# jwmak/ceres-solver-cuda

Hardware: AMD Instinct MI355X
Metric: residual+Jacobian evaluations/sec on BAL problem-13682; achieved HBM GB/s (higher is better)
Workload: dtype f64

## Files before the change

__graft_entry__.py:

```python
import os
import subprocess
import sys

REPO = os.path.dirname(os.path.abspath(__file__))
PKG = os.path.join(REPO, "ceres-solver-cuda_amd")
for p in (PKG, os.path.join(REPO, "oracle"), os.path.join(REPO, "tests")):
    if p not in sys.path:
        sys.path.insert(0, p)


def build():
    jobs = str(min(16, os.cpu_count() or 1))
    subprocess.check_call(["make", "-j", jobs, "-C", PKG])
    subprocess.check_call(["make", "-j", jobs, "-C", os.path.join(REPO, "examples")])
    subprocess.check_call(["make", "-j", jobs, "-C", os.path.join(REPO, "oracle")])
    subprocess.check_call(["make", "-j", jobs, "-C", os.path.join(REPO, "tests", "hip")])
    subprocess.check_call(["make", "-j", jobs, "-C", os.path.join(REPO, "tests", "cpp"),
                           "all", "asan-cpu", "asan-hip"])
    subprocess.check_call(["make", "-j", jobs, "-C", os.path.join(REPO, "tests", "cpp"),
                           "-f", "per_block_loss.mk", "driver", "facade"])
    subprocess.check_call(["make", "-j", jobs, "-C", os.path.join(REPO, "tests", "cpp"),
                           "-f", "schur_pairs.mk", "driver"])
    subprocess.check_call(["make", "-j", jobs, "-C", os.path.join(REPO, "tests", "cpp"),
                           "-f", "schur_sparse.mk", "driver"])
    subprocess.check_call(["make", "-j", jobs, "-C", os.path.join(REPO, "tests", "cpp"),
                           "-f", "cg_state.mk", "driver"])
    import ceres_amd
    from ceres_amd import _cse
    _cse.lib()
    return ceres_amd


def smoke():
    import numpy as np
    import torch

    import ceres_amd as ca
    from ceres_amd import bal
    import oracle_py as O
    from parity_util import assert_parity

    assert torch.cuda.is_available(), "smoke() needs a HIP device"
    prog = bal.synthetic_program((16, 2000, 7600), loss=ca.Loss.huber(1.0), seed=11)
    ev = ca.Evaluator(prog, device=0)
    got = ev.evaluate()
    info = ev.info()
    ev.close()
    op = O.OracleProgram.from_program(prog)
    ref = op.evaluate(prog.state, num_threads=4)
    assert_parity(got, ref, "smoke")
    assert info.num_affine_groups == 1
    print(f"smoke ok: cost {got[1]:.12e} (oracle {ref[1]:.12e}), "
          f"{prog.num_residual_blocks} blocks, {prog.num_jacobian_values} Jacobian values")
    return True


if __name__ == "__main__":
    build()
    if len(sys.argv) > 1 and sys.argv[1] == "smoke":
# ... 2 lines not shown
```

ceres-solver-cuda_amd/ceres_amd/_cse.py:

```python
import ctypes as C
import os

HERE = os.path.dirname(os.path.abspath(__file__))
LIB_PATH = os.path.normpath(os.path.join(HERE, "..", "lib", "libcse.so"))

CSE_ABI_VERSION = 6

JACOBIAN_CLOSED_FORM = 0
JACOBIAN_JET = 1
CSE_OK = 0
CSE_EVALUATION_FAILED = 1
CSE_ERR_INVALID = -1
CSE_ERR_HIP = -2
CSE_ERR_OOM = -3
CSE_ERR_UNSUPPORTED = -4
EVAL_SAME_POINT = 1

SNAVELY_2_9_3 = 0
SNAVELY_NO_DISTORTION_2_7_3 = 1
SNAVELY_QUATERNION_2_10_3 = 2
POINT_DISPLACEMENT_3_3 = 3
TEST_LINEAR_3_2_3_4 = 100
TEST_LINEAR_3_4_3_2 = 101
TEST_LINEAR_2_2_3 = 102
# ... 138 lines not shown
    "cse_set_plus_jacobians": (C.c_int, [C.c_void_p, P_f64]),
    "cse_plus_device": (C.c_int, [C.c_void_p, C.c_void_p, C.c_void_p, C.c_void_p]),
    "cse_plus": (C.c_int, [C.c_void_p, P_f64, P_f64, P_f64]),
    "cse_jacobian_right_multiply": (C.c_int, [C.c_void_p, C.c_void_p, C.c_void_p, C.c_void_p]),
    "cse_jacobian_left_multiply": (C.c_int, [C.c_void_p, C.c_void_p, C.c_void_p, C.c_void_p]),
    "cse_cgnr_multiply": (C.c_int, [C.c_void_p, C.c_void_p, C.c_void_p, C.c_void_p, C.c_void_p]),
    "cse_jacobian_squared_column_norm": (C.c_int, [C.c_void_p, C.c_void_p, C.c_void_p]),
    "cse_jacobian_scale_columns": (C.c_int, [C.c_void_p, C.c_void_p, C.c_void_p]),
    "cse_schur_structure": (C.c_int, [C.c_void_p, P_i64, P_i64]),
    "cse_schur_init": (C.c_int, [C.c_void_p, C.c_void_p, C.c_void_p, C.c_void_p, C.c_void_p,
                                 C.c_int]),
    "cse_schur_init_gradient": (C.c_int, [C.c_void_p, C.c_void_p, C.c_void_p, C.c_void_p,
                                          C.c_void_p, C.c_int, C.c_void_p]),
    "cse_schur_multiply": (C.c_int, [C.c_void_p, C.c_void_p, C.c_void_p]),
    "cse_schur_precondition": (C.c_int, [C.c_void_p, C.c_void_p, C.c_void_p]),
    "cse_schur_back_substitute": (C.c_int, [C.c_void_p, C.c_void_p, C.c_void_p]),
    "cse_schur_complement": (C.c_int, [C.c_void_p, C.c_void_p, C.c_int64]),
    "cse_schur_complement_plan": (C.c_int, [C.c_void_p, P_i64, P_i64, P_i64]),
    "cse_schur_complement_sparse_structure": (C.c_int, [C.c_void_p, P_i64, P_i64, P_i64, P_i64, P_i32]),
    "cse_schur_complement_sparse": (C.c_int, [C.c_void_p, C.c_void_p]),
    "cse_schur_explicit_multiply": (C.c_int, [C.c_void_p, C.c_void_p, C.c_void_p, C.c_void_p]),
    "cse_cg_default_options": (None, [C.POINTER(cse_cg_options)]),
    "cse_schur_solve": (C.c_int, [C.c_void_p, C.POINTER(cse_cg_options), C.c_void_p, C.c_void_p,
                                  C.c_void_p, C.c_void_p, C.POINTER(cse_cg_summary)]),
    "cse_create_multi": (C.c_int, [C.POINTER(cse_problem_desc), C.POINTER(cse_options),
                                   P_i32, C.c_int32, C.POINTER(C.c_void_p)]),
    "cse_shard_info": (C.c_int, [C.c_void_p, P_i32, P_i64, P_i32]),
    "cse_shard_transfer_bytes": (C.c_int, [C.c_void_p, P_i64, P_i64]),
    "cse_host_register": (C.c_int, [C.c_void_p, C.c_size_t]),
    "cse_host_unregister": (C.c_int, [C.c_void_p]),
    "cse_destroy": (None, [C.c_void_p]),
    "cse_last_error": (C.c_char_p, []),
    "cse_get_info": (C.c_int, [C.c_void_p, C.POINTER(cse_info)]),
    "cse_kernel_stats": (C.c_int, [C.c_void_p, P_f64, P_f64, P_i64]),
    "cse_reset_kernel_stats": (C.c_int, [C.c_void_p]),
    "cse_block_sparse_layout": (C.c_int, [C.c_int64, P_pb, C.c_int64, P_i64, P_i32, P_i32,
                                          C.c_int64, P_i64, P_i64, P_i64, P_i64]),
    "cse_compressed_row_layout": (C.c_int, [C.c_int64, P_pb, C.c_int64, P_i64, P_i32, P_i32,
                                            P_i64, P_i64, P_i64, P_i64, P_i64, P_i64]),
    "cse_layout_offsets_count": (C.c_int64, [C.c_int64, P_pb, C.c_int64, P_i64, P_i32, P_i32]),
    "cse_register_functor": (C.c_int, [C.c_void_p, P_i32]),
    "cse_functor_shape": (C.c_int, [C.c_int32, P_i32, P_i32, P_i32, P_i32]),
    "cse_abi_version": (C.c_int, []),
    "cse_build_info": (C.c_char_p, []),
}

_SINCE_ROUND3 = {"cse_evaluate_ex", "cse_evaluate_device_ex"}
_DEFAULT_LIB = LIB_PATH

_lib = None


def use_library(path):
    global LIB_PATH
    if _lib is not None:
        raise RuntimeError("libcse already loaded from " + LIB_PATH)
    LIB_PATH = os.path.abspath(path)


def lib():
    global _lib
    if _lib is None:
        if not os.path.exists(LIB_PATH):
            raise RuntimeError(
                f"libcse.so not found at {LIB_PATH}: build it with `make -C "
                f"ceres-solver-cuda_amd` (there is no CPU fallback)")
        handle = C.CDLL(LIB_PATH)
        for name, (res, args) in SIGNATURES.items():
            if name in _SINCE_ROUND3 and LIB_PATH != _DEFAULT_LIB and not hasattr(handle, name):
                continue
            fn = getattr(handle, name)
            fn.restype = res
            fn.argtypes = args
        if handle.cse_abi_version() != CSE_ABI_VERSION:
            raise RuntimeError("libcse.so ABI version mismatch")
        _lib = handle
    return _lib


def cg_options(**fields):
    o = cse_cg_options()
    lib().cse_cg_default_options(C.byref(o))
    for k, v in fields.items():
        if k not in dict(cse_cg_options._fields_):
            raise TypeError(f"cse_cg_options has no field {k}")
        setattr(o, k, v)
    return o


def last_error():
    return lib().cse_last_error().decode()


def functor_shape(kind):
    if kind in FUNCTOR_SHAPES:
        return FUNCTOR_SHAPES[kind]
    nr, nb, d = C.c_int32(), C.c_int32(), C.c_int32()
    sizes = (C.c_int32 * MAX_PARAMETER_BLOCKS)()
    check(lib().cse_functor_shape(int(kind), C.byref(nr), C.byref(nb), sizes, C.byref(d)),
          "cse_functor_shape")
    shape = (nr.value, tuple(sizes[:nb.value]), d.value)
    FUNCTOR_SHAPES[kind] = shape
# ... 13 lines not shown
```

ceres-solver-cuda_amd/ceres_amd/problem.py:

```python
import ctypes as C
from dataclasses import dataclass, field
from typing import List, Optional

import numpy as np

from . import _cse
from ._cse import FUNCTOR_SHAPES, functor_shape

BLOCK_SPARSE = "block_sparse"
COMPRESSED_ROW = "compressed_row"


def _ptr(a, ctype):
    if a is None:
        return None
    return a.ctypes.data_as(C.POINTER(ctype))


@dataclass
class Loss:
    kind: int = _cse.LOSS_TRIVIAL
    a: float = 1.0
    scaled: bool = False
    scale: float = 1.0
# ... 436 lines not shown
        forms = {"closed": _cse.JACOBIAN_CLOSED_FORM, "jet": _cse.JACOBIAN_JET}
        if jacobian_form not in forms:
            raise ValueError(f"jacobian_form must be one of {sorted(forms)}")
        opts.jacobian_form = forms[jacobian_form]
        opts.use_stream = int(stream is not None)
        opts.stream = stream if stream else None
        h = C.c_void_p()
        if devices is None:
            _cse.check(L.cse_create(C.byref(self.desc), C.byref(opts), C.byref(h)), "cse_create")
        else:
            if stream is not None:
                raise ValueError("a multi-device evaluator runs on its own per-device streams")
            devs = (C.c_int32 * len(devices))(*devices)
            _cse.check(L.cse_create_multi(C.byref(self.desc), C.byref(opts), devs, len(devices),
                                          C.byref(h)), "cse_create_multi")
        self.handle = h

    def close(self):
        if getattr(self, "handle", None):
            _cse.lib().cse_destroy(self.handle)
            self.handle = None

    def __del__(self):
        try:
            self.close()
        except Exception:
            pass

    def info(self):
        inf = _cse.cse_info()
        _cse.check(_cse.lib().cse_get_info(self.handle, C.byref(inf)), "cse_get_info")
        return inf

    def shard_info(self):
        L = _cse.lib()
        n = C.c_int32()
        _cse.check(L.cse_shard_info(self.handle, C.byref(n), None, None), "cse_shard_info")
        first = np.empty(n.value + 1, np.int64)
        devs = np.empty(n.value, np.int32)
        _cse.check(L.cse_shard_info(self.handle, C.byref(n), _ptr(first, C.c_int64),
                                    _ptr(devs, C.c_int32)), "cse_shard_info")
        return first, devs

    def transfer_bytes(self):
        first, _ = self.shard_info()
        n = len(first) - 1
        h2d = np.empty(n, np.int64)
        d2h = np.empty(n, np.int64)
        _cse.check(_cse.lib().cse_shard_transfer_bytes(self.handle, _ptr(h2d, C.c_int64),
                                                        _ptr(d2h, C.c_int64)),
                   "cse_shard_transfer_bytes")
        return h2d, d2h

    def evaluate(self, state=None, residuals=True, gradient=True, jacobian=True, out=None,
                 new_evaluation_point=True):
        p = self.program
        state = np.ascontiguousarray(p.state if state is None else state, np.float64)
        cost = C.c_double(-1.0)
        ro, go, jo = out if out is not None else (None, None, None)
        r = (ro if ro is not None else np.empty(p.num_residuals)) if residuals else None
        g = (go if go is not None else np.empty(p.num_effective_parameters)) if gradient else None
        j = (jo if jo is not None else np.empty(p.num_jacobian_values)) if jacobian else None
        flags = 0 if new_evaluation_point else _cse.EVAL_SAME_POINT
        rc = _cse.lib().cse_evaluate_ex(self.handle, _ptr(state, C.c_double), C.byref(cost),
                                        _ptr(r, C.c_double), _ptr(g, C.c_double),
                                        _ptr(j, C.c_double), flags)
# ... 140 lines not shown
```

ceres-solver-cuda_amd/csrc/cse_evaluator.hip:

```cpp
#include <hip/hip_runtime.h>

#include <algorithm>
#include <cmath>
#include <cstdio>
#include <cstdlib>
#include <cstring>
#include <mutex>
#include <new>
#include <string>
#include <type_traits>
#include <utility>
#include <vector>

#include "../../include/cse.h"
#include "evaluation_kernels.hpp"
#include "evaluator.hpp"
#include "group_store_kernel.hpp"
#include "jet_kernels.h"
#include "kernel_pickers.hpp"
#include "launch.hpp"
#include "multi_device.h"
#include "per_block_loss_kernels.h"
#include "plan.hpp"

// ... 132 lines not shown
    a.jac_stride[j] = G.jac_stride[j];
    for (int r = 0; r < 3; ++r) a.jac_base[j][r] = G.jac_base[j][r];
  }
  a.res_base = G.res_base;
  a.packed0 = G.packed0.p;
  a.packed0_lo = G.slot0_lo;
  a.packed0_stride = G.packed_stride;
  a.act0_bits = G.act0.p;
  a.fbase = G.fbase.p;
  a.side = G.side.p;
  a.delta0 = G.delta0.p;
  a.gindex = G.gindex.p;
  a.first = G.first;
  a.residual_layout = ev->res_layout.p;
  a.jac_layout = ev->jac_layout.p;
  a.jac_offsets = ev->jac_offsets.p;
  a.residuals = res;
  a.jacobian = jac;
  a.gradient = grad;
  a.partials = ev->partials.p + G.partial_offset;
  a.status = ev->status.p;
  a.loss.a = G.loss.a;
  a.loss.scale = G.loss.scale;
  a.loss.scaled = G.loss.scaled;
  static_assert(sizeof(a.user_loss) == sizeof(G.loss.user), "user loss bytes");
  std::memcpy(a.user_loss, G.loss.user, sizeof(a.user_loss));
  a.apply_loss = ev->opts.apply_loss_function;
  a.check_finite = ev->opts.check_finite;
  a.table_runs = G.runs.p;
  a.plain0 = G.plain0 ? 1 : 0;
  a.plain0_state_base = G.plain0_state_base;
  a.plain0_delta_base = G.plain0_delta_base;
  a.loss_data = G.loss_data.p;
  return a;
}

cse::GradArgs SlotGradArgs(const Group& G, int j, const double* jac, const double* res, double* grad) {
  const Group::GradPlan& P = G.grad[j];
  cse::GradArgs ga{};
  ga.jac = jac;
  for (int r = 0; r < G.shape.nr && r < 3; ++r) ga.jrow[r] = G.jac_base[j][r];
  ga.jstride = G.jac_stride[j];
  ga.res = res;
  ga.res_base = G.res_base;
  ga.perm = P.perm.p;
  ga.off = P.off.p;
  ga.count = P.count;
  ga.lo = P.lo;
  ga.grad = grad;
  ga.delta_base = G.delta_base[j];
  return ga;
}

int LaunchContribReduce(const Group::GradPlan& P, const double* gcontrib, const cse::GradArgs& ga,
                        hipStream_t s) {
  const cse::GradChunks ch = GradChunksOf(P);
  if (P.nchunks > 0)
    hipLaunchKernelGGL((cse::GradientContribKernel<9, 10>),
                       dim3((unsigned)((P.nchunks + cse::kWavesPerBlock - 1) / cse::kWavesPerBlock)),
                       dim3(cse::kBlockThreads), 0, s, gcontrib, P.perm.p, ch, P.chunk_order.p);
  hipLaunchKernelGGL((cse::GradientChunkReduceKernel<9>),
                     dim3((unsigned)((ga.count + cse::kBlockThreads - 1) / cse::kBlockThreads)),
                     dim3(cse::kBlockThreads), 0, s, ga, ch);
  CSE_HIP(hipGetLastError());
  return CSE_OK;
}
// ... 124 lines not shown
    return Fail(CSE_ERR_UNSUPPORTED, "fused gradient: slot 0 of " + std::to_string(G.shape.s0) + " parameters");
  CSE_HIP(hipGetLastError());
  return CSE_OK;
}

int UploadGroup(const cse_residual_group& g, const cse::GroupTables& T, Group* Gp, hipStream_t s) {
  Group& G = *Gp;
  const KindShape& k = G.shape;
  int rc;
  if (G.repack0 && (rc = G.packed0.alloc((size_t)G.slot0_count * G.packed_stride))) return rc;
  if ((rc = G.act0.upload(T.bits.data(), T.bits.size(), s))) return rc;
  if ((rc = G.src0.upload(T.src.data(), T.src.size(), s))) return rc;
  if ((rc = G.delta0.upload(T.dlt.data(), T.dlt.size(), s))) return rc;
  if ((rc = G.fbase.upload(T.fbase.data(), T.fbase.size(), s))) return rc;
  if ((rc = G.prev_seg.upload(T.prev_seg.data(), T.prev_seg.size(), s))) return rc;
  if ((rc = G.side.alloc(T.prev_seg.size() * 16))) return rc;
  for (int j = 0; j < 2; ++j) {
    Group::GradPlan& D = G.grad[j];
    const cse::GradTables& H = T.grad[j];
    static_cast<cse::GradPlanInfo&>(D) = T.grad_info[j];
    if ((rc = D.perm.upload(H.perm.data(), H.perm.size(), s))) return rc;
    if ((rc = D.off.upload(H.off.data(), H.off.size(), s))) return rc;
    if ((rc = D.chunk_order.upload(H.chunk_order.data(), H.chunk_order.size(), s))) return rc;
    if ((rc = D.chunk_begin.upload(H.chunk_begin.data(), H.chunk_begin.size(), s))) return rc;
    if ((rc = D.chunk_off.upload(H.chunk_off.data(), H.chunk_off.size(), s))) return rc;
    if ((rc = D.chunk_pb.upload(H.chunk_pb.data(), H.chunk_pb.size(), s))) return rc;
    const int size = j == 0 ? k.s0 : k.s1;
    if (D.ready && !D.sorted &&
        (rc = D.chunk_partial.alloc((size_t)std::max<int64_t>(1, D.nchunks) * size)))
      return rc;
  }
  if ((rc = G.runs.upload(T.runs.data(), T.runs.size(), s))) return rc;
  if ((rc = G.ids.upload(g.parameter_block_ids, (size_t)g.num_blocks * k.nb, s))) return rc;
  std::vector<double> rows, records;
  if (G.loss_data_size) {
    const int64_t n = g.num_blocks, D = k.data, W = D + G.loss_data_size;
    rows.resize((size_t)(n * D));
    records.resize((size_t)(n * 2));
    for (int64_t i = 0; i < n; ++i) {
      for (int64_t c = 0; c < D; ++c) rows[i * D + c] = g.functor_data[i * W + c];
      records[2 * i] = g.functor_data[i * W + D];
      records[2 * i + 1] = g.functor_data[i * W + D + 1];
    }
    if ((rc = G.data.upload(rows.data(), rows.size(), s))) return rc;
    if ((rc = G.loss_data.upload(records.data(), records.size(), s))) return rc;
  } else if ((rc = G.data.upload(g.functor_data, (size_t)g.num_blocks * k.data, s))) {
    return rc;
  }
  if ((!G.affine || G.const0) && g.residual_block_index &&
      (rc = G.gindex.upload(g.residual_block_index, (size_t)g.num_blocks, s)))
    return rc;
  if (hipStreamSynchronize(s) != hipSuccess) return Fail(CSE_ERR_HIP, "upload failed");
  return CSE_OK;
}

struct GradPath {
  bool grad_pass = false, fused = false, recompute = false;
};
bool FusedGradMode(const cse_evaluator* ev, const Group& G) {
  const int mode = ev->opts.gradient_mode;
  return G.fuse_ok && (mode == 0 || (!G.user && ((mode == 3 && !G.jet) || (mode == 1 && G.const0))));
}
GradPath GradPathOf(const cse_evaluator* ev, const Group& G, bool grad, bool res, bool jac) {
  GradPath p;
  p.grad_pass = grad && res && jac && G.affine && ev->opts.gradient_mode != 2;
  for (int j = 0; j < G.shape.nb; ++j) p.grad_pass = p.grad_pass && G.grad[j].ready;
// ... 539 lines not shown

int cse_functor_shape(int32_t kind, int32_t* num_residuals, int32_t* num_parameter_blocks,
                      int32_t* parameter_block_sizes, int32_t* data_size) {
  KindShape k;
  if (!ShapeOf(kind, &k)) return Fail(CSE_ERR_UNSUPPORTED, "unknown functor kind " + std::to_string(kind));
  if (num_residuals) *num_residuals = k.nr;
  if (num_parameter_blocks) *num_parameter_blocks = k.nb;
  if (parameter_block_sizes)
    for (int j = 0; j < k.nb; ++j) parameter_block_sizes[j] = k.sz[j];
  if (data_size) *data_size = k.data;
  return CSE_OK;
}

int cse_get_info(cse_evaluator* ev, cse_info* info) {
  if (!ev || !info) return Fail(CSE_ERR_INVALID, "null argument");
  if (ev->multi) return MultiInfo(ev->multi, info);
  std::memset(info, 0, sizeof(*info));
  info->num_residual_blocks = ev->num_residual_blocks;
  info->num_residuals = ev->num_residuals;
  info->num_parameters = ev->num_parameters;
  info->num_effective_parameters = ev->num_effective;
  info->num_jacobian_values = ev->num_jacobian_values;
  info->num_groups = (int32_t)ev->groups.size();
  for (auto& G : ev->groups) {
    info->num_affine_groups += G.affine ? 1 : 0;
    info->num_fused_gradient_groups += FusedGradMode(ev, G) ? 1 : 0;
  }
  info->device = ev->device;
  info->bytes_jacobian_eval = ev->bytes_jac;
  info->bytes_residual_eval = ev->bytes_res;
  return CSE_OK;
}

int cse_kernel_stats(cse_evaluator* ev, double* last_ms, double* total_ms, int64_t* launches) {
  if (!ev) return Fail(CSE_ERR_INVALID, "null evaluator");
  if (ev->multi) return MultiKernelStats(ev->multi, last_ms, total_ms, launches);
  if (!ev->opts.profile) return Fail(CSE_ERR_INVALID, "evaluator created without options.profile");
  int rc = FoldTiming(ev);
  if (rc) return rc;
  if (last_ms) *last_ms = ev->last_ms;
  if (total_ms) *total_ms = ev->total_ms;
  if (launches) *launches = ev->launches;
  return CSE_OK;
}

int cse_reset_kernel_stats(cse_evaluator* ev) {
  if (!ev) return Fail(CSE_ERR_INVALID, "null evaluator");
  if (ev->multi) return MultiResetKernelStats(ev->multi);
  int rc = FoldTiming(ev);
  if (rc) return rc;
  ev->last_ms = ev->total_ms = 0.0;
  ev->launches = 0;
  return CSE_OK;
}

}
```

ceres-solver-cuda_amd/csrc/evaluate_kernel.hpp:

```cpp
#ifndef CSE_EVALUATE_KERNEL_HPP_
#define CSE_EVALUATE_KERNEL_HPP_

#include <type_traits>

#include "kernel_common.hpp"

namespace cse {

template <class K, bool kJac, bool kCrs, bool kHalves = false, bool kConst0 = false>
__device__ __forceinline__ void StageAndStore(const GroupArgs& a, double* st, int lane, bool active,
                                              int64_t i0, int nw, const double* r,
                                              const double* J0, const double* J1,
                                              bool act0 = true, int64_t c = 0) {
  using Tr = KindTraits<K>;
  constexpr int NR = Tr::NR, NB = Tr::NB, S0 = Tr::S0, S1 = Tr::S1, S1p = Tr::S1p;
  constexpr int N = S0 + S1;
  if (nw <= 0) return;
  if (a.residuals && active) {
    double* dst = a.residuals + a.res_base + (int64_t)NR * (i0 + lane);
#pragma unroll
    for (int k = 0; k < NR; ++k) __builtin_nontemporal_store(r[k], dst + k);
  }
  if constexpr (kJac) {
    if (!a.jacobian) return;
// ... 96 lines not shown
  }
}

template <int kR, int kCols>
__device__ __forceinline__ void AddGradientSlot(double* g, int t, const double* r, const double* J) {
#pragma unroll
  for (int c = 0; c < kCols; ++c) {
    if (c >= t) break;
    double s = 0.0;
#pragma unroll
    for (int k = 0; k < kR; ++k) s += J[k * kCols + c] * r[k];
    unsafeAtomicAdd(g + c, s);
  }
}

template <class K>
struct AffineInputs {
  double d[KindTraits<K>::D];
  double x0[KindTraits<K>::X0];
  double x0pad;
  double x1[KindTraits<K>::S1p];
  int32_t id0, id1;
};

template <class K>
__device__ __forceinline__ int2 LoadIds(const GroupArgs& a, int64_t i) {
  if constexpr (KindTraits<K>::NB == 2) {
    return *reinterpret_cast<const int2*>(a.ids + 2 * i);
  } else {
    return make_int2(a.ids[i], 0);
  }
}

template <class K, bool kNtLoads>
__device__ __forceinline__ void GatherDataAndSlot1(const GroupArgs& a, int64_t i, int2 id,
                                                   AffineInputs<K>* in) {
  using Tr = KindTraits<K>;
  constexpr int S1 = Tr::S1, D = Tr::D;
  if constexpr (kNtLoads) {
#pragma unroll
    for (int k = 0; k < D; ++k) in->d[k] = __builtin_nontemporal_load(a.data + i * D + k);
  } else if constexpr (D == 2) {
    const double2 v = *reinterpret_cast<const double2*>(a.data + 2 * i);
    in->d[0] = v.x;
    in->d[1] = v.y;
  } else {
#pragma unroll
    for (int k = 0; k < D; ++k) in->d[k] = a.data[i * D + k];
  }
  if constexpr (S1 > 0) {
    const double* p1 = a.state + a.state_base[1] + (int64_t)S1 * id.y;
#pragma unroll
    for (int k = 0; k < S1; ++k) in->x1[k] = kNtLoads ? __builtin_nontemporal_load(p1 + k) : p1[k];
  }
}

template <class K>
__device__ __forceinline__ void GatherCoop(const GroupArgs& a, int64_t i, int2 id,
                                           AffineInputs<K>* in, double* lds, int lane) {
  constexpr int X0 = KindTraits<K>::X0;
  GatherDataAndSlot1<K, false>(a, i, id, in);
  const double* base0 = a.state + a.state_base[0];
  double piece[X0];
#pragma unroll
  for (int k = 0; k < X0; ++k) {
    const int p = k * kWave + lane;
// ... 10 lines not shown
  in->id0 = id.x;
  in->id1 = id.y;
}

template <class K>
__device__ __forceinline__ void GatherCoopDma(const GroupArgs& a, int64_t i, int2 id,
                                              AffineInputs<K>* in, double* lds, int lane) {
  using Tr = KindTraits<K>;
  constexpr int X0 = Tr::X0;
  constexpr int X0p = (X0 + 1) & ~1;
  constexpr int kPieces = X0p / 2;
  constexpr int kRow = PackedRowDoubles(X0);
  const int cid_own = id.x - a.packed0_lo;
#pragma unroll
  for (int k = 0; k < kPieces; ++k) {
    const int p = k * kWave + lane;
    const int t = p / kPieces, q = p - t * kPieces;
    const int cid = __shfl(cid_own, t, kWave);
    const double* src = a.packed0 + (int64_t)kRow * cid + 2 * q;
    __builtin_amdgcn_global_load_lds(src, lds + 2 * kWave * k, 16, 0, 0);
  }
  GatherDataAndSlot1<K, true>(a, i, id, in);
  asm volatile("s_waitcnt vmcnt(0)" ::: "memory");
  __builtin_amdgcn_wave_barrier();
#pragma unroll
  for (int k = 0; k < X0; ++k) in->x0[k] = lds[lane * X0p + k];
  if constexpr (X0 < X0p) in->x0pad = lds[lane * X0p + X0];
  __builtin_amdgcn_wave_barrier();
  in->id0 = id.x;
  in->id1 = id.y;
}

template <class K>
__device__ __forceinline__ void GatherEarly(const GroupArgs& a, int64_t i, int2 id,
                                            AffineInputs<K>* in, double* lds, int lane) {
  using Tr = KindTraits<K>;
  constexpr int X0 = Tr::X0, S1 = Tr::S1, D = Tr::D;
  constexpr int X0p = (X0 + 1) & ~1;
  constexpr int kPieces = X0p / 2;
  static_assert(D == 2, "observation pairs");
  const double obs_x = __builtin_nontemporal_load(a.data + 2 * i);
  const double obs_y = __builtin_nontemporal_load(a.data + 2 * i + 1);
  const int cid_own = id.x - a.packed0_lo;
#pragma unroll
  for (int k = 0; k < kPieces; ++k) {
    const int p = k * kWave + lane;
    const int t = p / kPieces, q = p - t * kPieces;
    const int cid = __shfl(cid_own, t, kWave);
    const double* src = a.packed0 + (int64_t)PackedRowDoubles(X0) * cid + 2 * q;
    __builtin_amdgcn_global_load_lds(src, lds + 2 * kWave * k, 16, 0, 0);
  }
  if constexpr (S1 > 0) {
    const double* p1 = a.state + a.state_base[1] + (int64_t)S1 * id.y;
#pragma unroll
    for (int k = 0; k < S1; ++k) in->x1[k] = __builtin_nontemporal_load(p1 + k);
  }
  in->d[0] = obs_x;
  in->d[1] = obs_y;
  asm volatile("s_waitcnt vmcnt(0)" ::: "memory");
  __builtin_amdgcn_wave_barrier();
#pragma unroll
  for (int k = 0; k < X0; ++k) in->x0[k] = lds[lane * X0p + k];
  __builtin_amdgcn_wave_barrier();
  in->id0 = id.x;
  in->id1 = id.y;
}

template <int S>
__device__ __forceinline__ void SegmentedScan(double* v, int key, int lane) {
#pragma unroll
  for (int off = 1; off < kWave; off <<= 1) {
    const int ku = __shfl_up(key, off, kWave);
    double vu[S];
#pragma unroll
    for (int c = 0; c < S; ++c) vu[c] = __shfl_up(v[c], off, kWave);
// ... 192 lines not shown
                          : kCrs ? kStageMinLaneCrs : kStageMinLane;
  constexpr int kStageLane = kPadLane > kStageLane1 ? kPadLane : kStageLane1;
  __shared__ double stage[kWPB][kWave * kStageLane];

  constexpr bool kC0J = T::kConst0 && kJac;
  const int lane = threadIdx.x & (kWave - 1);
  const int wave = kWPB == 1 ? 0 : threadIdx.x / kWave;
  const int64_t num_chunks = (a.n + kWave - 1) / kWave;
  const int64_t c = (int64_t)blockIdx.x * kWPB + wave;
  double* partial_dst = a.partials + c;
  if (c >= num_chunks) {
    if (lane == 0) *partial_dst = 0.0;
    return;
  }
  double* st = stage[wave];
  const int64_t i0 = c * kWave;
  const int64_t rem = a.n - i0;
  const int nw = rem < kWave ? (int)rem : kWave;
  const bool active = lane < nw;
  const int64_t i = active ? i0 + lane : a.n - 1;
  int64_t fb[5] = {0, 0, 0, 0, 0};
  if constexpr (kC0J) {
    fb[0] = a.fbase[c];
    fb[1] = a.fbase[c + 1];
    fb[2] = a.fbase[0];
    fb[3] = a.fbase[num_chunks];
    fb[4] = a.fbase[c + 2 < num_chunks ? c + 2 : num_chunks];
  }

  AffineInputs<K> in;
  LossParams lp;
  LoadBlockLoss<kLoss, kCoop == 2>(a, i, &lp);
  if constexpr (kCoop == 2) {
    int2 id;
    if constexpr (Tr::NB == 2) {
      const long long b = __builtin_nontemporal_load(reinterpret_cast<const long long*>(a.ids) + i);
      id = make_int2((int)b, (int)(b >> 32));
    } else {
      id = LoadIds<K>(a, i);
    }
    if constexpr (!kJac && Tr::D == 2 && Tr::NB == 2) {
      GatherEarly<K>(a, i, id, &in, st, lane);
    } else {
      GatherCoopDma<K>(a, i, id, &in, st, lane);
    }
  } else {
    GatherCoop<K>(a, i, LoadIds<K>(a, i), &in, st, lane);
  }
  if constexpr (kC0J) {
    if constexpr (kWPB == 1)
      asm volatile("" : "+s"(fb[0]), "+s"(fb[1]), "+s"(fb[2]), "+s"(fb[3]), "+s"(fb[4]));
    else
      asm volatile("" : "+v"(fb[0]), "+v"(fb[1]), "+v"(fb[2]), "+v"(fb[3]), "+v"(fb[4]));
  }
  double r[NR], J0[NR * S0], J1[NR * S1p];
  bool ok = EvaluateFunctor<K, kJac>(in.d, in.x0, in.x1, r, J0, J1);
  if (ok && a.check_finite) {
    bool bad = AnyNonFinite<NR>(r);
    if constexpr (kJac) bad = bad || AnyNonFinite<NR * S0>(J0) || AnyNonFinite<NR * S1>(J1);
    ok = !bad;
  }
  const double cost =
      LossAndCorrect<K, kLoss, kJac>(LossOf<kLoss>(a, lp), a.apply_loss, r, J0, J1, a.residuals != nullptr,
                                     a.user_loss);
  bool act0 = true;
  if constexpr (T::kConst0) {
    static_assert(kCoop == 2, "constant slot-0 blocks: the repacked table");
    if constexpr ((Tr::X0 & 1) != 0) {
      act0 = in.x0pad == 0.0;
    } else {
      const uint32_t k0 = (uint32_t)(in.id0 - a.packed0_lo);
      act0 = ((a.act0_bits[k0 >> 5] >> (k0 & 31)) & 1u) != 0;
    }
  }
  if (kJac && a.gradient != nullptr && active) {
    if (act0)
// ... 933 lines not shown
```

ceres-solver-cuda_amd/csrc/evaluator.hpp:

```cpp
#ifndef CSE_EVALUATOR_HPP_
#define CSE_EVALUATOR_HPP_

#include <hip/hip_runtime.h>

#include <cstdint>
#include <string>
#include <utility>
#include <vector>

#include "../../include/cse.h"
#include "cg_state.hpp"
#include "plan.hpp"

struct CseMulti;

namespace cse {

struct GroupArgs;
struct GradArgs;

inline int Fail(int code, const std::string& msg) { return CseFail(code, msg); }

#define CSE_SINGLE_DEVICE(ev, what)                                                         \
  do {                                                                                     \
// ... 32 lines not shown
    if (count == 0) return CSE_OK;
    if (hipMalloc(&p, count * sizeof(T)) != hipSuccess) {
      p = nullptr;
      return Fail(CSE_ERR_OOM, "hipMalloc of " + std::to_string(count * sizeof(T)) + " bytes failed");
    }
    n = count;
    return CSE_OK;
  }
  int ensure(size_t count) {
    if (p && n >= count) return CSE_OK;
    return alloc(count);
  }
  int upload(const T* h, size_t count, hipStream_t s) {
    int rc = alloc(count);
    if (rc) return rc;
    if (count && hipMemcpyAsync(p, h, count * sizeof(T), hipMemcpyHostToDevice, s) != hipSuccess)
      return Fail(CSE_ERR_HIP, "hipMemcpyAsync H2D failed");
    return CSE_OK;
  }
  void release() {
    if (p) (void)hipFree(p);
    p = nullptr;
    n = 0;
  }
};

struct Group : cse::GroupPlan {
  std::string user_name;
  DevBuf<int32_t> ids;
  DevBuf<double> data;
  DevBuf<double> loss_data;
  DevBuf<int64_t> gindex;
  DevBuf<double> packed0;
  struct GradPlan : cse::GradPlanInfo {
    DevBuf<int32_t> perm;
    DevBuf<int64_t> off;
    DevBuf<int64_t> chunk_begin, chunk_off;
    DevBuf<int32_t> chunk_pb;
    DevBuf<int32_t> chunk_order;
    DevBuf<double> chunk_partial;
  } grad[2];
  DevBuf<uint32_t> act0;
  DevBuf<int64_t> src0, fbase, delta0;
  DevBuf<double> side;
  DevBuf<int32_t> prev_seg;
  DevBuf<double> gside, gcontrib;
  DevBuf<double> sdata;
  DevBuf<int32_t> sid1;
  bool sorted_ready = false;
  DevBuf<int64_t> runs;
};

constexpr int kOperatorWavesPerWg = cse::kWavesPerBlock;

inline bool SnavelyShaped(const Group& G) { return cse::SnavelyShaped(G.shape); }
inline bool UserFused(const Group& G) { return cse::UserFused(G.user, G.shape); }

}

struct cse_evaluator {
  CseMulti* multi = nullptr;
  int device = 0;
  int num_cus = 256;
  hipStream_t stream = nullptr;
  bool own_stream = false;
  cse_options opts{};
// ... 73 lines not shown
```

ceres-solver-cuda_amd/csrc/host_shared.hpp:

```cpp
#ifndef CSE_HOST_SHARED_HPP_
#define CSE_HOST_SHARED_HPP_

#include <stdint.h>

namespace cse {

constexpr int kBlockThreads = 256;
constexpr int kWave = 64;
constexpr int kWavesPerBlock = kBlockThreads / kWave;
constexpr int kMaxSlots = 10;

constexpr int64_t kPlusJacobianQuaternion = -2;
struct PbDev {
  int64_t state_offset;
  int64_t delta_offset;
  int64_t plus_jacobian_offset;
  int32_t tangent_size;
  int32_t is_constant;
};

constexpr int PackedRowDoubles(int s) {
  const int p = (s + 1) & ~1;
  return p <= 2 ? 2 : p <= 4 ? 4 : p <= 8 ? 8 : p <= 16 ? 16 : p;
}

constexpr int kGradChunk = 512;

struct PlusRun {
  int64_t state_begin;
  int64_t length;
  int64_t delta_shift;
};

struct QuatPlusBlock {
  int64_t state_offset;
  int64_t delta_offset;
  int32_t size;
  int32_t pad;
};

constexpr int kTableRunFlagResiduals = 1, kTableRunFlagBsm = 2, kTableRunFlagCrs = 4;

}

#endif
```

ceres-solver-cuda_amd/csrc/kernel_common.hpp:

```cpp
#ifndef CSE_KERNEL_COMMON_HPP_
#define CSE_KERNEL_COMMON_HPP_

#include <stdint.h>

#include "functors.hpp"
#include "host_shared.hpp"
#include "jet.hpp"
#include "loss.hpp"

namespace cse {

constexpr double kImpossibleValue = 1e302;

struct GroupArgs {
  int64_t n;
  const int32_t* ids;
  const double* data;
  const double* state;
  const double* cstate;
  const PbDev* pbs;
  const double* plus_jacobians;
  int64_t state_base[2];
  int64_t delta_base[2];
  int64_t res_base;
  int64_t jac_base[2][3];
  int64_t jac_stride[2];
  const double* packed0;
  int32_t packed0_lo;
  int32_t packed0_stride;
  const uint32_t* act0_bits;
  const int64_t* fbase;
  double* side;
  const int64_t* delta0;
  const int64_t* gindex;
  int64_t first;
  const int64_t* residual_layout;
  const int64_t* jac_layout;
  const int64_t* jac_offsets;
  double* residuals;
  double* jacobian;
  double* gradient;
  double* partials;
  int* status;
  double* gfused;
  double* gside;
  double* gcontrib;
  LossParams loss;
  int apply_loss;
  int check_finite;
  double user_loss[kUserLossDoubles];
  const int64_t* table_runs;
  int64_t plain0_state_base, plain0_delta_base;
  int32_t plain0;
  const double* loss_data;
};

constexpr uint64_t kGroupArgsTag = 0x6373654761310006ull;

template <class K>
constexpr int SlotOffset(int j) {
  int o = 0;
  for (int b = 0; b < j; ++b) o += K::kSizes[b];
  return o;
}
template <class K>
constexpr int MaxSlotSize() {
  int m = 0;
  for (int b = 0; b < K::kNumBlocks; ++b) m = K::kSizes[b] > m ? K::kSizes[b] : m;
  return m;
}
template <class K, class = void>
struct Ambient0 {
  static constexpr int value = K::kSize0;
};
template <class K>
struct Ambient0<K, decltype((void)K::kAmbient0)> {
  static constexpr int value = K::kAmbient0;
};
template <class K>
struct KindTraits {
  static constexpr int NR = K::kNumResiduals;
  static constexpr int NB = K::kNumBlocks;
  static constexpr int S0 = K::kSize0;
  static constexpr int X0 = Ambient0<K>::value;
  static constexpr int S1 = NB > 1 ? K::kSize1 : 0;
  static constexpr int S1p = S1 > 0 ? S1 : 1;
  static constexpr int D = K::kDataSize;
  static constexpr int N = SlotOffset<K>(NB);
  static constexpr int Size(int j) { return K::kSizes[j]; }
  static constexpr int Off(int j) { return SlotOffset<K>(j); }
// ... 266 lines not shown
```

ceres-solver-cuda_amd/csrc/plan.cpp:

```cpp
#include "plan.hpp"

#include <algorithm>
#include <cmath>
#include <new>
#include <utility>

namespace cse {
std::string& LastError();
}

int CseFail(int code, const std::string& msg) {
  cse::LastError() = msg;
  return code;
}

namespace cse {

namespace {

int Fail(int code, const std::string& msg) { return CseFail(code, msg); }

bool GradSupported(int nr, int size, const cse_functor_ops* user, int slot) {
  if (user) return user->gradient[slot] != nullptr;
  return (nr == 2 && (size == 9 || size == 3 || size == 7 || size == 10)) || (nr == 3 && size == 3);
// ... 629 lines not shown
  S.f_cols = f_hi - f_lo;
  S.f_col_base = G.delta_base[0] - S.e_cols;
  std::vector<int64_t>& ranges = P->schur_chunk_begin;
  std::vector<int64_t>& big = P->schur_big;
  std::vector<int32_t> cams;
  bool dup = false;
  int64_t run_start = 0, chunk_lo = 0;
  for (int64_t i = 1; i <= n; ++i) {
    if (i < n && ids[2 * i + 1] == ids[2 * (i - 1) + 1]) continue;
    const int64_t len = i - run_start;
    cams.assign(len, 0);
    for (int64_t q = 0; q < len; ++q) cams[q] = ids[2 * (run_start + q)];
    std::sort(cams.begin(), cams.end());
    dup = dup || std::adjacent_find(cams.begin(), cams.end()) != cams.end();
    if (len > kWave) {
      if (run_start > chunk_lo) ranges.insert(ranges.end(), {chunk_lo, run_start});
      big.insert(big.end(), {run_start, i});
      chunk_lo = i;
    } else if (i - chunk_lo > kWave) {
      ranges.insert(ranges.end(), {chunk_lo, run_start});
      chunk_lo = run_start;
    }
    run_start = i;
  }
  if (n > chunk_lo) ranges.insert(ranges.end(), {chunk_lo, n});
  S.duplicates = dup;
  S.nchunks = (int64_t)ranges.size() / 2;
  S.nbig = (int64_t)big.size() / 2;
  S.eligible = true;
}

}

void PlanGroup(const cse_problem_desc* d, const cse_options& opts, int gi, ProgramPlan* P,
               GroupPlan* Gp, GroupTables* T) {
  const cse_residual_group& g = d->groups[gi];
  *Gp = GroupPlan{};
  *T = GroupTables{};
  GroupPlan& G = *Gp;
  G.kind = g.functor_kind;
  G.user = P->users[gi];
  G.shape = P->shapes[gi];
  G.loss = g.loss;
  G.loss_data_size = g.loss_data_size;
  G.n = g.num_blocks;
  G.first = g.first_residual_block;
  const KindShape& k = G.shape;

  G.policy = opts.force_general_layout ? kTable : DetectAffine(d, g, k, &G, T);
  if (G.policy != kTable && G.const0 && G.slot0_count > (1 << 20)) G.policy = kTable;
  G.jet = opts.jacobian_form == CSE_JACOBIAN_JET && g.functor_kind == CSE_FUNCTOR_SNAVELY_2_9_3;
  if (G.jet && G.policy != kTable &&
      (G.const0 || G.slot0_count <= 0 || G.slot0_count > (1 << 20)))
    G.policy = kTable;
  G.affine = G.policy != kTable;
  if (!G.affine) {
    G.const0 = false;
    T->fbase.clear();
  }
  if (G.affine && g.functor_kind == CSE_FUNCTOR_SNAVELY_QUATERNION_2_10_3 &&
      G.slot0_manifold == CSE_MANIFOLD_QUATERNION_EUCLIDEAN) {
    G.kind = kKindQuaternionTangent;
    ShapeOf(G.kind, nullptr, &G.shape);
  }
  if (G.const0 || !G.affine) P->any_general = true;

  if (G.affine) {
    const int64_t chunks = (g.num_blocks + kWave - 1) / kWave;
    G.num_wg = std::max<int64_t>(1, (chunks + kWavesPerBlock - 1) / kWavesPerBlock);
  } else {
    G.num_wg = (g.num_blocks + kBlockThreads - 1) / kBlockThreads;
  }
  G.partial_offset = P->total_wg;
  P->total_wg += G.num_wg * kWavesPerBlock;

  G.repack0 = G.affine && G.slot0_count > 0 && G.slot0_count <= (1 << 20);
  if (G.const0) {
    BuildConst0Tables(d, G, T);
    if (!T->fbase.empty()) G.fbase0 = T->fbase[0];
  }
  const bool fused_kind = FusedKind(G.kind) || UserFused(G.user, k);
  if (G.affine && P->has_layout) {
    const int sizes[2] = {k.s0, k.s1};
    for (int j = 0; j < k.nb; ++j)
      if (GradSupported(k.nr, sizes[j], G.user, j))
        BuildGradPlan(g, k, j, &T->grad_info[j], &T->grad[j],
                      j == 0 && G.const0 ? d->parameter_blocks : nullptr,
                      j == 0 && k.nb == 2 && fused_kind ? CamGradPasses(g, k) : 1);
  }
  BuildTableRuns(d, g, G, P->has_layout, &T->runs);
  DetectPlain0(d, g, &G);

  const GradPlanInfo* I = T->grad_info;
  bool ok = fused_kind && G.affine && G.n > 0 && G.repack0 && I[0].ready && !I[0].sorted &&
            I[0].nchunks > 0 && I[1].ready && I[1].sorted;
  for (int64_t i = 0; ok && i < g.num_blocks; ++i)
    ok = P->owner[g.parameter_block_ids[2 * i + 1]] == 2 * gi + 1;
  G.fuse_ok = ok;
  G.grad_exact = ok && d->num_groups == 1 && !G.const0 && d->num_constant_parameters == 0 &&
                 k.s1 == 3 && I[0].all_present && I[1].all_present &&
                 k.s0 * I[0].count + 3 * I[1].count == d->num_effective_parameters;
}

void PlanProgram(const cse_problem_desc* d, const GroupPlan* only, ProgramPlan* P) {
  std::vector<std::pair<int64_t, int64_t>> blocks;
  for (int64_t b = 0; b < d->num_parameter_blocks; ++b) {
    const cse_parameter_block& pb = d->parameter_blocks[b];
    if (pb.is_constant) continue;
    if (pb.manifold == CSE_MANIFOLD_QUATERNION_EUCLIDEAN) {
      P->plus_quat.push_back({pb.state_offset, pb.delta_offset, pb.size, 0});
      continue;
    }
    if (pb.plus_jacobian_offset >= 0 || pb.tangent_size != pb.size) P->plus_supported = false;
// ... 163 lines not shown
```

ceres-solver-cuda_amd/csrc/plan.hpp:

```cpp
#ifndef CSE_PLAN_HPP_
#define CSE_PLAN_HPP_

#include <stdint.h>

#include <string>
#include <vector>

#include "../../include/cse.h"
#include "host_shared.hpp"

int CseFail(int code, const std::string& msg);

namespace cse {

enum Policy { kTable = 0, kAffinePacked = 1, kAffineCrs = 2 };

constexpr int kKindQuaternionTangent = -100;

struct KindShape {
  int nr = 0, nb = 0, data = 0;
  int sz[kMaxSlots] = {};
  int s0 = 0, s1 = 0;
  int x0 = 0;
};
// ... 64 lines not shown
void BuildGradPlan(const cse_residual_group& g, const KindShape& k, int j, GradPlanInfo* plan,
                   GradTables* tables, const cse_parameter_block* cpb = nullptr, int passes = 1);

struct GroupPlan {
  int kind = 0;
  const cse_functor_ops* user = nullptr;
  KindShape shape{};
  cse_loss loss{};
  int loss_data_size = 0;
  int64_t n = 0;
  bool affine = false;
  int policy = 0;
  int64_t partial_offset = 0;
  int64_t num_wg = 0;
  int64_t first = 0;
  int64_t state_base[2] = {0, 0};
  int64_t delta_base[2] = {0, 0};
  int64_t res_base = 0;
  int64_t jac_base[2][3] = {{0, 0, 0}, {0, 0, 0}};
  int64_t jac_stride[2] = {0, 0};
  bool repack0 = false;
  int32_t slot0_lo = 0;
  int64_t slot0_count = 0;
  int slot0_stride = 0;
  int packed_stride = 0;
  int slot0_manifold = CSE_MANIFOLD_MATRIX;
  bool grad_exact = false;
  bool const0 = false;
  int64_t fbase0 = 0;
  bool fuse_ok = false;
  bool jet = false;
  bool plain0 = false;
  int64_t plain0_state_base = 0, plain0_delta_base = 0;
};

struct GroupTables {
  std::vector<uint32_t> bits;
  std::vector<int64_t> src, dlt, fbase;
  std::vector<int32_t> prev_seg;
  std::vector<int64_t> runs;
  GradPlanInfo grad_info[2];
  GradTables grad[2];
};

struct SchurPlan {
  bool eligible = false;
  bool duplicates = false;
  int64_t e_cols = 0, f_cols = 0;
  int64_t f_col_base = 0;
  int64_t nchunks = 0, nbig = 0;
};

struct ProgramPlan {
  bool has_layout = false;
  std::vector<KindShape> shapes;
  std::vector<const cse_functor_ops*> users;
  std::vector<std::string> user_names;
  std::vector<int32_t> owner;
  bool res_covered = true, jac_covered = true;
  int64_t bytes_jac = 0, bytes_res = 0;
  int64_t total_wg = 0;
  bool any_general = false;
  bool plus_supported = true;
  std::vector<PlusRun> plus_runs;
  std::vector<QuatPlusBlock> plus_quat;
  SchurPlan schur;
  std::vector<int64_t> schur_chunk_begin, schur_big;
  std::vector<PbDev> pbs;
};

int Validate(const cse_problem_desc* d);
int ValidateLossData(const cse_problem_desc* d, const cse_options* opts);
int ValidateGroups(const cse_problem_desc* d, UserLookup lookup, ProgramPlan* P,
                   const cse_options* opts = nullptr);

void PlanGroup(const cse_problem_desc* d, const cse_options& opts, int gi, ProgramPlan* P,
// ... 49 lines not shown
```

include/cse.h:

```cpp
#ifndef CSE_H_
#define CSE_H_

#include <stddef.h>
#include <stdint.h>

#ifdef __cplusplus
extern "C" {
#endif

#define CSE_ABI_VERSION 6

#define CSE_OK 0
#define CSE_EVALUATION_FAILED 1
#define CSE_ERR_INVALID -1
#define CSE_ERR_HIP -2
#define CSE_ERR_OOM -3
#define CSE_ERR_UNSUPPORTED -4

typedef enum cse_functor_kind {
  CSE_FUNCTOR_SNAVELY_2_9_3 = 0,
  CSE_FUNCTOR_SNAVELY_NO_DISTORTION_2_7_3 = 1,
  CSE_FUNCTOR_SNAVELY_QUATERNION_2_10_3 = 2,
  CSE_FUNCTOR_POINT_DISPLACEMENT_3_3 = 3,
  CSE_FUNCTOR_TEST_LINEAR_3_2_3_4 = 100,
// ... 256 lines not shown

int cse_create_multi(const cse_problem_desc* desc, const cse_options* options,
                     const int32_t* devices, int32_t num_devices, cse_evaluator** out);

int cse_shard_info(cse_evaluator* ev, int32_t* num_shards, int64_t* first_block,
                   int32_t* devices);

int cse_shard_transfer_bytes(cse_evaluator* ev, int64_t* state_h2d_bytes,
                             int64_t* strips_d2h_bytes);

int cse_host_register(void* p, size_t bytes);
int cse_host_unregister(void* p);

void cse_destroy(cse_evaluator* ev);

const char* cse_last_error(void);

typedef struct cse_info {
  int64_t num_residual_blocks;
  int64_t num_residuals;
  int64_t num_parameters;
  int64_t num_effective_parameters;
  int64_t num_jacobian_values;
  int32_t num_groups;
  int32_t num_affine_groups;
  int32_t device;
  int32_t num_fused_gradient_groups;
  int64_t bytes_jacobian_eval;
  int64_t bytes_residual_eval;
} cse_info;

int cse_get_info(cse_evaluator* ev, cse_info* info);

int cse_kernel_stats(cse_evaluator* ev, double* last_ms, double* total_ms,
                     int64_t* launches);
int cse_reset_kernel_stats(cse_evaluator* ev);

int cse_block_sparse_layout(int64_t num_parameter_blocks,
                            const cse_parameter_block* parameter_blocks,
                            int64_t num_residual_blocks, const int64_t* param_begin,
                            const int32_t* param_ids, const int32_t* num_residuals,
                            int64_t num_eliminate_blocks, int64_t* residual_layout,
                            int64_t* jacobian_per_residual_layout,
                            int64_t* jacobian_per_residual_offsets,
                            int64_t* num_jacobian_values);
int cse_compressed_row_layout(int64_t num_parameter_blocks,
                              const cse_parameter_block* parameter_blocks,
                              int64_t num_residual_blocks, const int64_t* param_begin,
                              const int32_t* param_ids, const int32_t* num_residuals,
                              int64_t* residual_layout,
                              int64_t* jacobian_per_residual_layout,
                              int64_t* jacobian_per_residual_offsets,
                              int64_t* num_jacobian_values, int64_t* crs_rows,
                              int64_t* crs_cols);
int64_t cse_layout_offsets_count(int64_t num_parameter_blocks,
                                 const cse_parameter_block* parameter_blocks,
                                 int64_t num_residual_blocks, const int64_t* param_begin,
                                 const int32_t* param_ids, const int32_t* num_residuals);

int cse_abi_version(void);
const char* cse_build_info(void);

#ifdef __cplusplus
}
#endif

// ... 2 lines not shown
```

Measured before the change: 780.7.

## Add compact 16-bit camera / run-mask block index for two-slot groups

Result: no change. 778.3 (-0.3%).

```diff
diff --git a/__graft_entry__.py b/__graft_entry__.py
--- a/__graft_entry__.py
+++ b/__graft_entry__.py
@@ -25,6 +25,8 @@
                            "-f", "schur_sparse.mk", "driver"])
     subprocess.check_call(["make", "-j", jobs, "-C", os.path.join(REPO, "tests", "cpp"),
                            "-f", "cg_state.mk", "driver"])
+    subprocess.check_call(["make", "-j", jobs, "-C", os.path.join(REPO, "tests", "cpp"),
+                           "-f", "compact_index.mk", "driver"])
     import ceres_amd
     from ceres_amd import _cse
     _cse.lib()
diff --git a/ceres-solver-cuda_amd/ceres_amd/_cse.py b/ceres-solver-cuda_amd/ceres_amd/_cse.py
--- a/ceres-solver-cuda_amd/ceres_amd/_cse.py
+++ b/ceres-solver-cuda_amd/ceres_amd/_cse.py
@@ -194,6 +194,7 @@
     "cse_destroy": (None, [C.c_void_p]),
     "cse_last_error": (C.c_char_p, []),
     "cse_get_info": (C.c_int, [C.c_void_p, C.POINTER(cse_info)]),
+    "cse_group_index_form": (C.c_int, [C.c_void_p, C.c_int]),
     "cse_kernel_stats": (C.c_int, [C.c_void_p, P_f64, P_f64, P_i64]),
     "cse_reset_kernel_stats": (C.c_int, [C.c_void_p]),
     "cse_block_sparse_layout": (C.c_int, [C.c_int64, P_pb, C.c_int64, P_i64, P_i32, P_i32,
@@ -208,6 +209,8 @@
 }
 
 _SINCE_ROUND3 = {"cse_evaluate_ex", "cse_evaluate_device_ex"}
+_SINCE_COMPACT_INDEX = {"cse_group_index_form"}
+_MAY_BE_MISSING = _SINCE_ROUND3 | _SINCE_COMPACT_INDEX
 _DEFAULT_LIB = LIB_PATH
 
 _lib = None
@@ -229,7 +232,7 @@
                 f"ceres-solver-cuda_amd` (there is no CPU fallback)")
         handle = C.CDLL(LIB_PATH)
         for name, (res, args) in SIGNATURES.items():
-            if name in _SINCE_ROUND3 and LIB_PATH != _DEFAULT_LIB and not hasattr(handle, name):
+            if name in _MAY_BE_MISSING and LIB_PATH != _DEFAULT_LIB and not hasattr(handle, name):
                 continue
             fn = getattr(handle, name)
             fn.restype = res
diff --git a/ceres-solver-cuda_amd/ceres_amd/problem.py b/ceres-solver-cuda_amd/ceres_amd/problem.py
--- a/ceres-solver-cuda_amd/ceres_amd/problem.py
+++ b/ceres-solver-cuda_amd/ceres_amd/problem.py
@@ -492,6 +492,10 @@
         _cse.check(_cse.lib().cse_get_info(self.handle, C.byref(inf)), "cse_get_info")
         return inf
 
+    def group_index_form(self, group=0):
+        return _cse.check(_cse.lib().cse_group_index_form(self.handle, int(group)),
+                          "cse_group_index_form")
+
     def shard_info(self):
         L = _cse.lib()
         n = C.c_int32()
diff --git a/ceres-solver-cuda_amd/csrc/cse_evaluator.hip b/ceres-solver-cuda_amd/csrc/cse_evaluator.hip
--- a/ceres-solver-cuda_amd/csrc/cse_evaluator.hip
+++ b/ceres-solver-cuda_amd/csrc/cse_evaluator.hip
@@ -188,6 +188,8 @@
   a.plain0_state_base = G.plain0_state_base;
   a.plain0_delta_base = G.plain0_delta_base;
   a.loss_data = G.loss_data.p;
+  a.cam16 = G.compact ? G.cam16.p : nullptr;
+  a.chunk_desc = G.compact ? G.chunk_desc.p : nullptr;
   return a;
 }
 
@@ -378,6 +380,8 @@
   }
   if ((rc = G.runs.upload(T.runs.data(), T.runs.size(), s))) return rc;
   if ((rc = G.ids.upload(g.parameter_block_ids, (size_t)g.num_blocks * k.nb, s))) return rc;
+  if ((rc = G.cam16.upload(T.cam16.data(), T.cam16.size(), s))) return rc;
+  if ((rc = G.chunk_desc.upload(T.chunk_desc.data(), T.chunk_desc.size(), s))) return rc;
   std::vector<double> rows, records;
   if (G.loss_data_size) {
     const int64_t n = g.num_blocks, D = k.data, W = D + G.loss_data_size;
@@ -983,6 +987,15 @@
   return CSE_OK;
 }
 
+int cse_group_index_form(cse_evaluator* ev, int group) {
+  if (!ev) return Fail(CSE_ERR_INVALID, "null evaluator");
+  CSE_SINGLE_DEVICE(ev, "cse_group_index_form");
+  if (group < 0 || group >= (int)ev->groups.size())
+    return Fail(CSE_ERR_INVALID, "group " + std::to_string(group) + " is not one of the evaluator's " +
+                                     std::to_string(ev->groups.size()));
+  return ev->groups[(size_t)group].compact ? 1 : 0;
+}
+
 int cse_kernel_stats(cse_evaluator* ev, double* last_ms, double* total_ms, int64_t* launches) {
   if (!ev) return Fail(CSE_ERR_INVALID, "null evaluator");
   if (ev->multi) return MultiKernelStats(ev->multi, last_ms, total_ms, launches);
diff --git a/ceres-solver-cuda_amd/csrc/evaluate_kernel.hpp b/ceres-solver-cuda_amd/csrc/evaluate_kernel.hpp
--- a/ceres-solver-cuda_amd/csrc/evaluate_kernel.hpp
+++ b/ceres-solver-cuda_amd/csrc/evaluate_kernel.hpp
@@ -152,6 +152,24 @@
   }
 }
 
+template <class K>
+__device__ __forceinline__ int2 LoadBlockIds(const GroupArgs& a, int64_t i, int64_t c) {
+  static_assert(KindTraits<K>::NB == 2, "two-slot kinds");
+  if (a.cam16 != nullptr) {
+    const int cam = __builtin_nontemporal_load(a.cam16 + i);
+    const uint32_t clo = __builtin_amdgcn_readfirstlane((uint32_t)c);
+    const uint32_t chi = __builtin_amdgcn_readfirstlane((uint32_t)((uint64_t)c >> 32));
+    const ChunkDesc* d = static_cast<const ChunkDesc*>(a.chunk_desc) + (((int64_t)chi << 32) | clo);
+    const int32_t first = d->first_point_id;
+    const uint64_t m = d->run_start_mask >> 1;
+    const int runs = (int)__builtin_amdgcn_mbcnt_hi((uint32_t)(m >> 32),
+                                                    __builtin_amdgcn_mbcnt_lo((uint32_t)m, 0u));
+    return make_int2(cam + a.packed0_lo, first + runs);
+  }
+  const long long b = __builtin_nontemporal_load(reinterpret_cast<const long long*>(a.ids) + i);
+  return make_int2((int)b, (int)(b >> 32));
+}
+
 template <class K, bool kNtLoads>
 __device__ __forceinline__ void GatherDataAndSlot1(const GroupArgs& a, int64_t i, int2 id,
                                                    AffineInputs<K>* in) {
@@ -228,15 +246,13 @@
 }
 
 template <class K>
-__device__ __forceinline__ void GatherEarly(const GroupArgs& a, int64_t i, int2 id,
-                                            AffineInputs<K>* in, double* lds, int lane) {
+__device__ __forceinline__ void GatherEarly(const GroupArgs& a, int64_t i, int2 id, double obs_x,
+                                            double obs_y, AffineInputs<K>* in, double* lds, int lane) {
   using Tr = KindTraits<K>;
   constexpr int X0 = Tr::X0, S1 = Tr::S1, D = Tr::D;
   constexpr int X0p = (X0 + 1) & ~1;
   constexpr int kPieces = X0p / 2;
   static_assert(D == 2, "observation pairs");
-  const double obs_x = __builtin_nontemporal_load(a.data + 2 * i);
-  const double obs_y = __builtin_nontemporal_load(a.data + 2 * i + 1);
   const int cid_own = id.x - a.packed0_lo;
 #pragma unroll
   for (int k = 0; k < kPieces; ++k) {
@@ -495,16 +511,18 @@
   LossParams lp;
   LoadBlockLoss<kLoss, kCoop == 2>(a, i, &lp);
   if constexpr (kCoop == 2) {
-    int2 id;
-    if constexpr (Tr::NB == 2) {
-      const long long b = __builtin_nontemporal_load(reinterpret_cast<const long long*>(a.ids) + i);
-      id = make_int2((int)b, (int)(b >> 32));
+    if constexpr (!kJac && Tr::D == 2 && Tr::NB == 2) {
+      const double obs_x = __builtin_nontemporal_load(a.data + 2 * i);
+      const double obs_y = __builtin_nontemporal_load(a.data + 2 * i + 1);
+      GatherEarly<K>(a, i, LoadBlockIds<K>(a, i, c), obs_x, obs_y, &in, st, lane);
     } else {
-      id = LoadIds<K>(a, i);
-    }
-    if constexpr (!kJac && Tr::D == 2 && Tr::NB == 2) {
-      GatherEarly<K>(a, i, id, &in, st, lane);
-    } else {
+      int2 id;
+      if constexpr (Tr::NB == 2) {
+        const long long b = __builtin_nontemporal_load(reinterpret_cast<const long long*>(a.ids) + i);
+        id = make_int2((int)b, (int)(b >> 32));
+      } else {
+        id = LoadIds<K>(a, i);
+      }
       GatherCoopDma<K>(a, i, id, &in, st, lane);
     }
   } else {
diff --git a/ceres-solver-cuda_amd/csrc/evaluator.hpp b/ceres-solver-cuda_amd/csrc/evaluator.hpp
--- a/ceres-solver-cuda_amd/csrc/evaluator.hpp
+++ b/ceres-solver-cuda_amd/csrc/evaluator.hpp
@@ -88,6 +88,8 @@
   DevBuf<double> loss_data;
   DevBuf<int64_t> gindex;
   DevBuf<double> packed0;
+  DevBuf<uint16_t> cam16;
+  DevBuf<cse::ChunkDesc> chunk_desc;
   struct GradPlan : cse::GradPlanInfo {
     DevBuf<int32_t> perm;
     DevBuf<int64_t> off;
diff --git a/ceres-solver-cuda_amd/csrc/host_shared.hpp b/ceres-solver-cuda_amd/csrc/host_shared.hpp
--- a/ceres-solver-cuda_amd/csrc/host_shared.hpp
+++ b/ceres-solver-cuda_amd/csrc/host_shared.hpp
@@ -24,6 +24,14 @@
   return p <= 2 ? 2 : p <= 4 ? 4 : p <= 8 ? 8 : p <= 16 ? 16 : p;
 }
 
+struct ChunkDesc {
+  int32_t first_point_id;
+  int32_t reserved;
+  uint64_t run_start_mask;
+};
+static_assert(sizeof(ChunkDesc) == 16, "one 16-byte record per chunk");
+constexpr int64_t kCompactMaxSlot0 = 65536;
+
 constexpr int kGradChunk = 512;
 
 struct PlusRun {
diff --git a/ceres-solver-cuda_amd/csrc/kernel_common.hpp b/ceres-solver-cuda_amd/csrc/kernel_common.hpp
--- a/ceres-solver-cuda_amd/csrc/kernel_common.hpp
+++ b/ceres-solver-cuda_amd/csrc/kernel_common.hpp
@@ -53,9 +53,11 @@
   int64_t plain0_state_base, plain0_delta_base;
   int32_t plain0;
   const double* loss_data;
-};
-
-constexpr uint64_t kGroupArgsTag = 0x6373654761310006ull;
+  const uint16_t* cam16;
+  const void* chunk_desc;
+};
+
+constexpr uint64_t kGroupArgsTag = 0x6373654761310007ull;
 
 template <class K>
 constexpr int SlotOffset(int j) {
diff --git a/ceres-solver-cuda_amd/csrc/plan.cpp b/ceres-solver-cuda_amd/csrc/plan.cpp
--- a/ceres-solver-cuda_amd/csrc/plan.cpp
+++ b/ceres-solver-cuda_amd/csrc/plan.cpp
@@ -685,6 +685,27 @@
 
 }
 
+bool BuildCompactIndex(const int32_t* ids, int64_t n, int32_t slot0_lo, int64_t slot0_count,
+                       std::vector<uint16_t>* cam16, std::vector<ChunkDesc>* chunk_desc) {
+  cam16->clear();
+  chunk_desc->clear();
+  if (n <= 0 || slot0_count <= 0 || slot0_count > kCompactMaxSlot0) return false;
+  for (int64_t i = 1; i < n; ++i) {
+    const int64_t step = (int64_t)ids[2 * i + 1] - ids[2 * i - 1];
+    if (step < 0 || step > 1) return false;
+  }
+  cam16->resize((size_t)n);
+  chunk_desc->assign((size_t)((n + kWave - 1) / kWave), ChunkDesc{0, 0, 0});
+  for (int64_t i = 0; i < n; ++i) {
+    (*cam16)[(size_t)i] = (uint16_t)(ids[2 * i] - slot0_lo);
+    ChunkDesc& c = (*chunk_desc)[(size_t)(i / kWave)];
+    const int l = (int)(i % kWave);
+    if (l == 0) c.first_point_id = ids[2 * i + 1];
+    else if (ids[2 * i + 1] != ids[2 * i - 1]) c.run_start_mask |= 1ull << l;
+  }
+  return true;
+}
+
 void PlanGroup(const cse_problem_desc* d, const cse_options& opts, int gi, ProgramPlan* P,
                GroupPlan* Gp, GroupTables* T) {
   const cse_residual_group& g = d->groups[gi];
@@ -732,6 +753,9 @@
     BuildConst0Tables(d, G, T);
     if (!T->fbase.empty()) G.fbase0 = T->fbase[0];
   }
+  G.compact = G.repack0 && !G.const0 && k.nb == 2 &&
+              BuildCompactIndex(g.parameter_block_ids, g.num_blocks, G.slot0_lo, G.slot0_count, &T->cam16,
+                                &T->chunk_desc);
   const bool fused_kind = FusedKind(G.kind) || UserFused(G.user, k);
   if (G.affine && P->has_layout) {
     const int sizes[2] = {k.s0, k.s1};
diff --git a/ceres-solver-cuda_amd/csrc/plan.hpp b/ceres-solver-cuda_amd/csrc/plan.hpp
--- a/ceres-solver-cuda_amd/csrc/plan.hpp
+++ b/ceres-solver-cuda_amd/csrc/plan.hpp
@@ -120,6 +120,7 @@
   bool jet = false;
   bool plain0 = false;
   int64_t plain0_state_base = 0, plain0_delta_base = 0;
+  bool compact = false;
 };
 
 struct GroupTables {
@@ -129,7 +130,20 @@
   std::vector<int64_t> runs;
   GradPlanInfo grad_info[2];
   GradTables grad[2];
-};
+  std::vector<uint16_t> cam16;
+  std::vector<ChunkDesc> chunk_desc;
+};
+
+bool BuildCompactIndex(const int32_t* ids, int64_t n, int32_t slot0_lo, int64_t slot0_count,
+                       std::vector<uint16_t>* cam16, std::vector<ChunkDesc>* chunk_desc);
+inline void DecodeCompactIndex(const uint16_t* cam16, const ChunkDesc* chunk_desc, int32_t slot0_lo,
+                               int64_t i, int32_t* id0, int32_t* id1) {
+  const ChunkDesc& c = chunk_desc[i / kWave];
+  const int l = (int)(i % kWave);
+  const uint64_t upto = l == kWave - 1 ? ~0ull : (2ull << l) - 1;
+  *id0 = (int32_t)cam16[i] + slot0_lo;
+  *id1 = c.first_point_id + __builtin_popcountll(c.run_start_mask & upto);
+}
 
 struct SchurPlan {
   bool eligible = false;
diff --git a/include/cse.h b/include/cse.h
--- a/include/cse.h
+++ b/include/cse.h
@@ -312,6 +312,8 @@
 
 int cse_get_info(cse_evaluator* ev, cse_info* info);
 
+int cse_group_index_form(cse_evaluator* ev, int group);
+
 int cse_kernel_stats(cse_evaluator* ev, double* last_ms, double* total_ms,
                      int64_t* launches);
 int cse_reset_kernel_stats(cse_evaluator* ev);
```
